# cosmir17/Scala-akka-tensorflow-sharetrade-helper

Measured on AMD Instinct MI355X. Metric: env steps/sec (whole node) + episode return, 2x128 MLP Q-net at 1/2/4/8 MI355X, higher is better.
Workload: dtype bf16; 1 GPU; model=2x128 MLP Q-net (203->128->128->3), online DQN, Adam, global_batch=1835008, seq_len=201, parallelism=dp1, dp_gradient_sync=none, envs_per_gpu=1835008, hip_graph=True, graph_steps=16, kernel_chunk=64, step_kernel=ws, chunk_schedule=static

## Files before the change

csrc/qtarget.hip:

```cpp
#include "qstep.h"

namespace st {
namespace qtgt {

constexpr int INP = 224, HP = 128, KX = 208, HWIN = 201;

constexpr int KS = 208;
constexpr int oW0 = 0;
constexpr int oW1 = oW0 + HP * KS * 2;
constexpr int oW2 = oW1 + HP * HP * 2;
constexpr int oB1 = oW2 + 4 * HP * 2;
constexpr int LDS_BYTES = oB1 + HP * 4;

ST_DEV int w1_off(int r, int c) { return r * HP + ((((c >> 3) ^ (r & 15))) << 3) + (c & 7); }
ST_DEV f4v mfma32z(s4v a, s4v b, f4v c) {
  const s4v z = {0, 0, 0, 0};
  return mfma32(cat8(a, z), cat8(b, z), c);
}
struct QTargetParams {
  const float* prices4;
  const int* env;
  const float* wt;
  float* qt;
  int T, E, T4;
  int off_w0, off_w1, off_b1, off_w2, off_b2;
  float b0, inv_b0;
  int s0, compat_env, output_relu, feat_mode;
  const unsigned char* wimg;
  const unsigned short* ticks;
  const float* tscale;
  int T16;
};

template <int FEAT, int TPW, int NWV, bool U16 = false>
__global__ void __launch_bounds__(64 * NWV, 1) qtarget_kernel(QTargetParams p) {
  static_assert(!U16 || FEAT, "the tick bank serves the relative features only");
  constexpr int NW = NWV, NT = 64 * NWV;
  extern __shared__ __attribute__((aligned(16))) char smem[];
  bf16_t* W0 = reinterpret_cast<bf16_t*>(smem + oW0);
  bf16_t* W1 = reinterpret_cast<bf16_t*>(smem + oW1);
  bf16_t* W2 = reinterpret_cast<bf16_t*>(smem + oW2);
  float* B1 = reinterpret_cast<float*>(smem + oB1);
  const int tid = threadIdx.x, lane = tid & 63, l16 = lane & 15, g4 = lane >> 4;
  const int w = tid >> 6;
  if (p.wimg != nullptr) {
    constexpr int NCH = LDS_BYTES / 16;
    const int lane_ = tid & 63;
    for (int j = tid >> 6; j * 64 < NCH; j += NW) {
      const int c = j * 64 + lane_;
      if (c < NCH)
        __builtin_amdgcn_global_load_lds((const __attribute__((address_space(1))) void*)(p.wimg + 16 * c),
                                         (__attribute__((address_space(3))) void*)(smem + 1024 * j), 16, 0, 0);
    }
    __builtin_amdgcn_s_waitcnt(0xF70);
  } else {
  for (int i = tid; i < HP * KX; i += NT) {
    const int r = i / KX, s = i % KX;
    W0[r * KS + s] = f2bf(p.wt[p.off_w0 + r * INP + slot_col(s)]);
  }
  for (int i = tid; i < HP * HP; i += NT) {
    const int r = i / HP, s = i % HP;
    W1[w1_off(r, s)] = f2bf(p.wt[p.off_w1 + r * HP + pi_unit(s)]);
  }
  for (int i = tid; i < 4 * HP; i += NT) {
    const int a = i / HP, s = i % HP;
    W2[i] = a < 3 ? f2bf(p.wt[p.off_w2 + a * HP + pi_unit(s)]) : (bf16_t)0;
  }
  for (int i = tid; i < HP; i += NT) B1[i] = p.wt[p.off_b1 + i];
  }
  __syncthreads();
  const float b2v[3] = {p.wt[p.off_b2], p.wt[p.off_b2 + 1], p.wt[p.off_b2 + 2]};
  const size_t E = (size_t)p.E;
  const int ntiles = p.E / 16;
  s4v w0t[8];
#pragma unroll
  for (int i = 0; i < 8; ++i) w0t[i] = lds_ld4(W0 + (16 * i + l16) * KS + 192 + 4 * g4);
  for (int t0 = (blockIdx.x * NW + w) * TPW; t0 < ntiles; t0 += gridDim.x * NW * TPW) {
    int zo = 0;
    asm volatile("" : "+s"(zo));
    const bf16_t* W0i = W0 + zo;
    float vnew[TPW], invn[TPW], vnw[TPW];
    Holding hd[TPW];
    s8v X[TPW][6];
    s4v Xw[TPW];
#pragma unroll
    for (int q = 0; q < TPW; ++q) {
      const int e = 16 * (t0 + q) + l16;
      const int pos = p.env[ER_POS * E + e];
      const float bud = __int_as_float(p.env[ER_BUDGET * E + e]);
      const int sh = p.env[ER_SHARES * E + e];
      const int pc = min(max(pos, 0), p.T - HWIN - 1);
      if (U16) {
        const unsigned* b = reinterpret_cast<const unsigned*>(p.ticks + (size_t)e * p.T16) + ((pc + 1) >> 1);
        const unsigned shb = (unsigned)((pc + 1) & 1) * 2u;
        const unsigned tv = __builtin_amdgcn_alignbyte(0u, b[100], shb);
        const float vw = (float)(tv & 0xFFFFu);
        vnew[q] = __fmul_rn(vw, p.tscale[e]);
        invn[q] = __fdiv_rn(1.0f, vw);
        vnw[q] = vw;
        const float iv = invn[q];
        auto fxn = [&](float v) { return __fmaf_rn(v, iv, -1.0f); };
        auto lo16f = [](unsigned v) { return (float)(v & 0xFFFFu); };
        auto hi16f = [](unsigned v) { return (float)(v >> 16); };
#pragma unroll
        for (int ks = 0; ks < 6; ++ks) {
          uint4 u;
          __builtin_memcpy(&u, b + 16 * ks + 4 * g4, sizeof(u));
          const unsigned t4 = b[16 * ks + 4 * g4 + 4];
          const unsigned w0 = __builtin_amdgcn_alignbyte(u.y, u.x, shb), w1 = __builtin_amdgcn_alignbyte(u.z, u.y, shb),
                         w2 = __builtin_amdgcn_alignbyte(u.w, u.z, shb), w3 = __builtin_amdgcn_alignbyte(t4, u.w, shb);
          X[q][ks] = cat8(pk4(fxn(lo16f(w0)), fxn(hi16f(w0)), fxn(lo16f(w1)), fxn(hi16f(w1))),
                          pk4(fxn(lo16f(w2)), fxn(hi16f(w2)), fxn(lo16f(w3)), fxn(hi16f(w3))));
        }
        Xw[q] = s4v{0, 0, 0, 0};
        if (g4 == 1 || g4 == 2) {
          uint2 u;
          __builtin_memcpy(&u, b + 96 + 2 * (g4 - 1), sizeof(u));
          const unsigned t2 = b[98 + 2 * (g4 - 1)];
          const unsigned w0 = __builtin_amdgcn_alignbyte(u.y, u.x, shb), w1 = __builtin_amdgcn_alignbyte(t2, u.y, shb);
          Xw[q] = pk4(fxn(lo16f(w0)), fxn(hi16f(w0)), fxn(lo16f(w1)), fxn(hi16f(w1)));
        }
      } else {
      const float* b = p.prices4 + (size_t)e * p.T4 + (size_t)pc;
      vnew[q] = b[201];
      vnw[q] = vnew[q];
      invn[q] = FEAT ? __fdiv_rn(1.0f, vnew[q]) : 0.f;
      const float iv = invn[q];
      auto fxn = [&](float v) { return FEAT ? __fmaf_rn(v, iv, -1.0f) : v; };
#pragma unroll
      for (int ks = 0; ks < 6; ++ks) {
        const float4 u = ldu4(b + 1 + 32 * ks + 8 * g4), v = ldu4(b + 5 + 32 * ks + 8 * g4);
        X[q][ks] = cat8(pk4(fxn(u.x), fxn(u.y), fxn(u.z), fxn(u.w)), pk4(fxn(v.x), fxn(v.y), fxn(v.z), fxn(v.w)));
      }
      Xw[q] = s4v{0, 0, 0, 0};
      if (g4 == 1 || g4 == 2) {
        const float4 u = ldu4(b + 193 + 4 * (g4 - 1));
        Xw[q] = pk4(fxn(u.x), fxn(u.y), fxn(u.z), fxn(u.w));
      }
      }
      hd[q] = trade_base(bud, sh, p.compat_env, p.b0, p.s0);
    }
    f4v a1[TPW][8];
#pragma unroll
    for (int i = 0; i < 8; ++i) {
#pragma unroll
      for (int q = 0; q < TPW; ++q) a1[q][i] = f4v{0.f, 0.f, 0.f, 0.f};
      const bf16_t* wr = W0i + (16 * i + l16) * KS + 8 * g4;
#pragma unroll
      for (int ks = 0; ks < 6; ++ks) {
        const s8v A = lds_ld8(wr + 32 * ks);
#pragma unroll
        for (int q = 0; q < TPW; ++q) a1[q][i] = mfma32(A, X[q][ks], a1[q][i]);
      }
#pragma unroll
      for (int q = 0; q < TPW; ++q) a1[q][i] = mfma32z(w0t[i], Xw[q], a1[q][i]);
    }
#pragma unroll 1
    for (int a = 0; a < 3; ++a) {
      int za = 0;
      asm volatile("" : "+s"(za));
      const bf16_t* W1a = W1 + za;
      const bf16_t* W2a = W2 + za;
      s8v H1[TPW][4];
#pragma unroll
      for (int q = 0; q < TPW; ++q) {
        const Holding h2 = trade(a, hd[q], vnew[q]);
        const float fvn = FEAT ? __fmaf_rn(vnw[q], invn[q], -1.0f) : vnew[q];
        const s4v tl = g4 == 0 ? pk4(feat_budget(h2.budget, p.inv_b0, FEAT),
                                     feat_shares(h2.shares, vnew[q], p.inv_b0, FEAT), 1.0f, fvn)
                               : s4v{0, 0, 0, 0};
#pragma unroll
        for (int ks = 0; ks < 4; ++ks) {
          const f4v z0 = mfma32z(w0t[2 * ks], tl, a1[q][2 * ks]);
          const f4v z1 = mfma32z(w0t[2 * ks + 1], tl, a1[q][2 * ks + 1]);
          H1[q][ks] = cat8(relu_bf(z0), relu_bf(z1));
        }
      }
      f4v qo[TPW];
#pragma unroll
      for (int q = 0; q < TPW; ++q) qo[q] = f4v{0.f, 0.f, 0.f, 0.f};
      const bf16_t* w2r = W2a + min(l16, 3) * HP + 8 * g4;
#pragma unroll
      for (int ks2 = 0; ks2 < 4; ++ks2) {
        f4v z[TPW][2];
#pragma unroll
        for (int h = 0; h < 2; ++h) {
          const int i = 2 * ks2 + h;
          const f4v bias = *reinterpret_cast<const f4v*>(B1 + 16 * i + 4 * g4);
#pragma unroll
          for (int q = 0; q < TPW; ++q) z[q][h] = bias;
#pragma unroll
          for (int ks = 0; ks < 4; ++ks) {
            const s8v A = lds_ld8(W1a + w1_off(16 * i + l16, 32 * ks + 8 * g4));
#pragma unroll
            for (int q = 0; q < TPW; ++q) z[q][h] = mfma32(A, H1[q][ks], z[q][h]);
          }
        }
        const s8v A2 = lds_ld8(w2r + 32 * ks2);
#pragma unroll
        for (int q = 0; q < TPW; ++q) qo[q] = mfma32(A2, cat8(relu_bf(z[q][0]), relu_bf(z[q][1])), qo[q]);
      }
      if (g4 == 0) {
#pragma unroll
        for (int q = 0; q < TPW; ++q) {
          float o[3];
#pragma unroll
          for (int j = 0; j < 3; ++j) {
            o[j] = qo[q][j] + b2v[j];
            if (p.output_relu) o[j] = fmaxf(o[j], 0.f);
          }
          const int e = 16 * (t0 + q) + l16;
          *reinterpret_cast<float4*>(p.qt + ((size_t)e * 3 + a) * 4) = make_float4(o[0], o[1], o[2], 0.f);
        }
      }
    }
  }
}

__global__ void __launch_bounds__(256) qt_img_map_kernel(int* map, int off_w0, int off_w1, int off_w2, int off_b1) {
  const int i = blockIdx.x * blockDim.x + threadIdx.x;
  if (i < HP * KX) map[off_w0 + (i / KX) * INP + slot_col(i % KX)] = oW0 / 2 + (i / KX) * KS + i % KX;
  if (i < HP * HP) map[off_w1 + (i / HP) * HP + pi_unit(i % HP)] = oW1 / 2 + w1_off(i / HP, i % HP);
  if (i < 3 * HP) map[off_w2 + (i / HP) * HP + pi_unit(i % HP)] = oW2 / 2 + i;
  if (i < HP) map[off_b1 + i] = -(oB1 / 4 + i) - 2;
}

}
}

extern "C" int st_qtarget_img_bytes() { return st::qtgt::LDS_BYTES; }

extern "C" hipError_t st_qtarget_img_map(int* map, int off_w0, int off_w1, int off_w2, int off_b1, hipStream_t stream) {
  using namespace st::qtgt;
  static_assert(LDS_BYTES % 16 == 0 && oW0 == 0, "image run");
  hipLaunchKernelGGL(qt_img_map_kernel, dim3((HP * KX + 255) / 256), dim3(256), 0, stream, map, off_w0, off_w1, off_w2,
                     off_b1);
  return hipGetLastError();
}


namespace {
template <int TPW, int NWV>
hipError_t launch_qt(const st::qtgt::QTargetParams* p, int grid, hipStream_t stream) {
  using namespace st::qtgt;
  if (p->E % (16 * TPW) != 0) return hipErrorInvalidValue;
  static bool attr[3] = {false, false, false};
  const bool u16 = p->ticks != nullptr;
  if (u16 && (!p->feat_mode || p->tscale == nullptr || p->T16 < p->T + 8 || p->T16 % 8)) return hipErrorInvalidValue;
  const int f = u16 ? 2 : (p->feat_mode ? 1 : 0);
  const void* fn = f == 2 ? (const void*)qtarget_kernel<1, TPW, NWV, true>
                          : (f ? (const void*)qtarget_kernel<1, TPW, NWV> : (const void*)qtarget_kernel<0, TPW, NWV>);
  if (!attr[f]) {
    hipError_t e = hipFuncSetAttribute(fn, hipFuncAttributeMaxDynamicSharedMemorySize, LDS_BYTES);
    if (e != hipSuccess) return e;
    attr[f] = true;
  }
  if (f == 2)
    hipLaunchKernelGGL((qtarget_kernel<1, TPW, NWV, true>), dim3(grid), dim3(64 * NWV), LDS_BYTES, stream, *p);
  else if (f)
    hipLaunchKernelGGL((qtarget_kernel<1, TPW, NWV>), dim3(grid), dim3(64 * NWV), LDS_BYTES, stream, *p);
  else
    hipLaunchKernelGGL((qtarget_kernel<0, TPW, NWV>), dim3(grid), dim3(64 * NWV), LDS_BYTES, stream, *p);
  return hipGetLastError();
}
}

extern "C" hipError_t st_qtarget_launch_v(const st::qtgt::QTargetParams* p, int grid, int variant, hipStream_t stream) {
  using namespace st::qtgt;
  if (grid < 1 || p->T < HWIN + 2 || p->T4 < p->T + 4) return hipErrorInvalidValue;
  switch (variant) {
    case 0: return launch_qt<4, 4>(p, grid, stream);
    case 1: return launch_qt<2, 8>(p, grid, stream);
    case 2: return launch_qt<1, 8>(p, grid, stream);
    case 3: return launch_qt<1, 16>(p, grid, stream);
    default: return hipErrorInvalidValue;
  }
}
extern "C" hipError_t st_qtarget_launch(const st::qtgt::QTargetParams* p, int grid, hipStream_t stream) {
  return st_qtarget_launch_v(p, grid, 1, stream);
}

extern "C" int st_abi_qtarget(int* out, int n) {
  const int sz[] = {(int)sizeof(st::QStepParams), (int)sizeof(st::qtgt::QTargetParams)};
  const int m = (int)(sizeof(sz) / sizeof(sz[0]));
  for (int i = 0; i < n && i < m; ++i) out[i] = sz[i];
  return m;
}
```

sharetrade/ops/native.py:

```python
from __future__ import annotations

import ctypes as C
import os
from typing import Optional

import torch

_HERE = os.path.dirname(os.path.abspath(__file__))
LIB_DIR = os.path.join(os.path.dirname(_HERE), "_native")
HIP_LIB_PATH = os.path.join(LIB_DIR, "libsharetrade_hip.so")

_lib: Optional[C.CDLL] = None


class NativeUnavailable(RuntimeError):
    pass


class QStepParams(C.Structure):
    _fields_ = [
        ("prices", C.c_void_p), ("prices4", C.c_void_p), ("env", C.c_void_p),
        ("wq", C.c_void_p), ("wf", C.c_void_p), ("slab", C.c_void_p), ("stats", C.c_void_p), ("ctrl", C.c_void_p),
        ("T", C.c_int), ("E", C.c_int), ("H", C.c_int), ("P", C.c_int), ("T4", C.c_int),
        ("off_w0", C.c_int), ("off_w1", C.c_int), ("off_b1", C.c_int), ("off_w2", C.c_int), ("off_b2", C.c_int),
        ("eps", C.c_float), ("inv_ramp", C.c_float), ("gamma", C.c_float), ("loss_coef", C.c_float),
        ("b0", C.c_float), ("inv_b0", C.c_float),
        ("s0", C.c_int), ("compat_env", C.c_int), ("target_compat", C.c_int), ("output_relu", C.c_int),
        ("feat_mode", C.c_int),
        ("key0", C.c_uint32), ("key1", C.c_uint32),
        ("env_offset", C.c_int),
        ("stamps", C.c_void_p),
        ("slab_bf16", C.c_int), ("slab_rows", C.c_int),
        ("chunk_heads", C.c_void_p),
        ("reward_mode", C.c_int), ("td_clip", C.c_float),
        ("err", C.c_void_p),
        ("reward_scale", C.c_float), ("ramp_global", C.c_int), ("qt", C.c_void_p), ("double_dqn", C.c_int),
        ("wimg", C.c_void_p),
        ("ticks", C.c_void_p), ("tscale", C.c_void_p), ("T16", C.c_int),
    ]


QTARGET_VARIANTS = {0: (4, 4), 1: (2, 8), 2: (1, 8), 3: (1, 16)}


class QTargetParams(C.Structure):
    _fields_ = [
        ("prices4", C.c_void_p), ("env", C.c_void_p), ("wt", C.c_void_p), ("qt", C.c_void_p),
        ("T", C.c_int), ("E", C.c_int), ("T4", C.c_int),
        ("off_w0", C.c_int), ("off_w1", C.c_int), ("off_b1", C.c_int), ("off_w2", C.c_int), ("off_b2", C.c_int),
        ("b0", C.c_float), ("inv_b0", C.c_float),
        ("s0", C.c_int), ("compat_env", C.c_int), ("output_relu", C.c_int), ("feat_mode", C.c_int),
        ("wimg", C.c_void_p),
        ("ticks", C.c_void_p), ("tscale", C.c_void_p), ("T16", C.c_int),
    ]


class OptimParams(C.Structure):
    _fields_ = [
        ("params", C.c_void_p), ("params_bf", C.c_void_p), ("mask", C.c_void_p), ("s1", C.c_void_p),
        ("s2", C.c_void_p), ("slab", C.c_void_p), ("grad", C.c_void_p), ("ctrl", C.c_void_p),
        ("stats", C.c_void_p), ("stat_acc", C.c_void_p),
        ("G", C.c_int), ("P", C.c_int), ("kind", C.c_int), ("mode", C.c_int), ("nstat", C.c_int),
        ("lr", C.c_float), ("beta1", C.c_float), ("beta2", C.c_float), ("eps", C.c_float), ("scale", C.c_float),
        ("tdelay", C.c_int), ("slab_bf16", C.c_int),
        ("chunk_heads", C.c_void_p),
        ("ema", C.c_void_p), ("ema_decay", C.c_float),
        ("img_map", C.c_void_p), ("img", C.c_void_p),
    ]


REWARD_MODES = {"absolute": 0, "relative": 1, "growth": 2}

ENV_ROWS = ("pos", "budget", "shares", "value", "ret_sum", "episodes", "last_final", "actions_out", "rewards_out")


AB_LIB_PATH = os.path.join(LIB_DIR, "libsharetrade_ab.so")
WRONG_RESULT_VARIANTS = frozenset({"gskip", "gskipst", "l1x2", "l2x2", "nopf", "nowb", "nophil"})
_ab_lib: Optional[C.CDLL] = None


def ab_builds_enabled() -> bool:
    return os.environ.get("SHARETRADE_AB_BUILDS", "") not in ("", "0")


def ab_lib() -> C.CDLL:
    global _ab_lib
    if not ab_builds_enabled():
        raise RuntimeError("timing / debug kernel builds are opt-in: set SHARETRADE_AB_BUILDS=1 and run "
                           "`python build.py --ab` (csrc/ab/*.hip -> libsharetrade_ab.so)")
    if _ab_lib is None:
        if not os.path.exists(AB_LIB_PATH):
            raise NativeUnavailable(f"{AB_LIB_PATH} not built: run `SHARETRADE_AB_BUILDS=1 python build.py`")
        lib()
        _ab_lib = C.CDLL(AB_LIB_PATH)
    return _ab_lib


def variant_launch(suffix: str, prefix: str = "st_qstep_ws_launch_"):
    if not ab_builds_enabled():
        bad = " (computes WRONG results by design)" if suffix in WRONG_RESULT_VARIANTS else ""
        raise RuntimeError(f"engine.step_variant={suffix!r}{bad} needs SHARETRADE_AB_BUILDS=1")
    fn = getattr(ab_lib(), prefix + suffix)
    fn.argtypes = [C.POINTER(QStepParams), C.c_int, C.c_int, C.c_int, C.c_int, C.c_void_p]
    fn.restype = C.c_int
    return fn


def available() -> bool:
    return os.path.exists(HIP_LIB_PATH)


def lib() -> C.CDLL:
    global _lib
    if _lib is not None:
        return _lib
    if not os.path.exists(HIP_LIB_PATH):
        raise NativeUnavailable(
            f"{HIP_LIB_PATH} not built: run `python build.py` (hipcc --offload-arch=gfx950)")
    L = C.CDLL(HIP_LIB_PATH)
    L.st_qstep_launch.argtypes = [C.POINTER(QStepParams), C.c_int, C.c_int, C.c_int, C.c_int, C.c_void_p]
    L.st_qstep_launch.restype = C.c_int
    L.st_qstep_lds_bytes.argtypes = [C.c_int, C.c_int, C.c_int]
    L.st_qstep_lds_bytes.restype = C.c_int
    L.st_qstep_wide_launch.argtypes = [C.POINTER(QStepParams), C.c_int, C.c_int, C.c_int, C.c_int, C.c_void_p]
    L.st_qstep_wide_launch.restype = C.c_int
    L.st_qstep_wide_lds_bytes.argtypes = [C.c_int, C.c_int, C.c_int]
    L.st_qstep_wide_lds_bytes.restype = C.c_int
    L.st_qstep_wide_launch_w8.argtypes = [C.POINTER(QStepParams), C.c_int, C.c_int, C.c_int, C.c_int, C.c_void_p]
    L.st_qstep_wide_launch_w8.restype = C.c_int
    L.st_qstep_ws_launch.argtypes = [C.POINTER(QStepParams), C.c_int, C.c_int, C.c_int, C.c_int, C.c_void_p]
    L.st_qstep_ws_launch.restype = C.c_int
    L.st_qstep_ws_lds_bytes.argtypes = [C.c_int, C.c_int, C.c_int]
    L.st_qstep_ws_lds_bytes.restype = C.c_int
    L.st_qtarget_launch.argtypes = [C.POINTER(QTargetParams), C.c_int, C.c_void_p]
    L.st_qtarget_launch.restype = C.c_int
    L.st_qtarget_launch_v.argtypes = [C.POINTER(QTargetParams), C.c_int, C.c_int, C.c_void_p]
    L.st_qtarget_launch_v.restype = C.c_int
    L.st_qtarget_img_bytes.argtypes = []
    L.st_qtarget_img_bytes.restype = C.c_int
    L.st_qtarget_img_map.argtypes = [C.c_void_p] + [C.c_int] * 4 + [C.c_void_p]
    L.st_qtarget_img_map.restype = C.c_int
    L.st_f32b_target_sync.argtypes = [C.c_void_p, C.c_void_p, C.c_longlong, C.c_void_p, C.c_longlong, C.c_void_p]
    L.st_f32b_target_sync.restype = C.c_int
    L.st_reduce_optim.argtypes = [C.POINTER(OptimParams), C.c_void_p]
    L.st_reduce_optim.restype = C.c_int
    L.st_advance.argtypes = [C.c_void_p, C.c_void_p]
    L.st_advance.restype = C.c_int
    L.st_commit_step.argtypes = [C.c_void_p, C.c_void_p]
    L.st_commit_step.restype = C.c_int
    L.st_to_bf16.argtypes = [C.c_void_p, C.c_void_p, C.c_int, C.c_void_p]
    L.st_to_bf16.restype = C.c_int
    L.st_img_pack.argtypes = [C.c_void_p, C.c_void_p, C.c_void_p, C.c_int, C.c_void_p]
    L.st_img_pack.restype = C.c_int
    L.st_qstep_ws_img_bytes.argtypes = []
    L.st_qstep_ws_img_bytes.restype = C.c_int
    L.st_qstep_ws_img_map.argtypes = [C.c_void_p] + [C.c_int] * 5 + [C.c_void_p]
    L.st_qstep_ws_img_map.restype = C.c_int
    L.st_random_walk.argtypes = [C.c_void_p, C.c_int, C.c_int, C.c_float, C.c_float, C.c_float, C.c_uint32,
                                 C.c_uint32, C.c_void_p]
    L.st_random_walk.restype = C.c_int
    L.st_replicate4.argtypes = [C.c_void_p, C.c_void_p, C.c_int, C.c_int, C.c_int, C.c_int, C.c_void_p]
    L.st_replicate4.restype = C.c_int
    L.st_tick16.argtypes = [C.c_void_p, C.c_int, C.c_int, C.c_void_p, C.c_int, C.c_void_p, C.c_int, C.c_void_p,
                            C.c_void_p]
    L.st_tick16.restype = C.c_int
    L.st_init_normal.argtypes = [C.c_void_p, C.c_int, C.c_int, C.c_int, C.c_float, C.c_uint32, C.c_uint32,
                                 C.c_uint32, C.c_void_p]
    L.st_init_normal.restype = C.c_int
    _bind_optional(L)
    _lib = L
    return L


def _bind_optional(L: C.CDLL) -> None:
    if hasattr(L, "st_occupy"):
        L.st_occupy.argtypes = [C.c_int, C.c_int, C.c_void_p, C.c_void_p]
        L.st_occupy.restype = C.c_int
    if hasattr(L, "st_tick_rcp_table"):
        L.st_tick_rcp_table.argtypes = [C.c_void_p, C.c_void_p, C.c_void_p]
        L.st_tick_rcp_table.restype = C.c_int
    if hasattr(L, "st_mlp_fwd_f32"):
        L.st_mlp_fwd_f32.restype = C.c_int
        L.st_td_update_f32.restype = C.c_int


def clear_last_error() -> int:
    return int(C.CDLL("libamdhip64.so").hipGetLastError())


def check(err: int, what: str) -> None:
    if err != 0:
        raise RuntimeError(f"HIP error {err} in {what}")


def ptr(t: Optional[torch.Tensor]) -> Optional[int]:
    if t is None:
        return None
    return t.data_ptr()


def stream_handle() -> int:
    return torch.cuda.current_stream().cuda_stream


def qstep_supported(inp: int, h1p: int, h2p: int) -> bool:
    if not available():
        return False
    return lib().st_qstep_lds_bytes(inp, h1p, h2p) > 0


def qstep_wide_supported(inp: int, h1p: int, h2p: int) -> bool:
    if not available():
        return False
    return lib().st_qstep_wide_lds_bytes(inp, h1p, h2p) > 0


def qstep_ws_supported(inp: int, h1p: int, h2p: int) -> bool:
    if not available():
        return False
    return lib().st_qstep_ws_lds_bytes(inp, h1p, h2p) > 0


def qstep_pipe_supported(inp: int, h1p: int, h2p: int) -> bool:
    if not available():
        return False
    fn = ab_lib().st_qstep_pipe_lds_bytes
    fn.argtypes = [C.c_int, C.c_int, C.c_int]
    fn.restype = C.c_int
    return fn(inp, h1p, h2p) > 0


def random_walk(out: torch.Tensor, start_price: float, vol: float, drift: float, key0: int, key1: int) -> None:
    E, T = out.shape
    check(lib().st_random_walk(ptr(out), E, T, start_price, vol, drift, key0 & 0xFFFFFFFF, key1 & 0xFFFFFFFF,
                               stream_handle()), "st_random_walk")


def replica_stride(T: int) -> int:
    return (T + 64 + 3) // 4 * 4


def replicate4(src: torch.Tensor, reps: int = 4) -> torch.Tensor:
    E, T = src.shape
    T4 = replica_stride(T)
    flat = torch.zeros(reps * E * T4 + 64, dtype=torch.float32, device=src.device)
    out = flat[: reps * E * T4].view(reps, E, T4)
    check(lib().st_replicate4(ptr(src), ptr(out), E, T, T4, int(reps), stream_handle()), "st_replicate4")
    return out


def tick16_stride(T: int) -> int:
    return (T + 8 + 7) // 8 * 8


def tick16(bank: torch.Tensor, quantize: bool):
    E, T = bank.shape
    if not bank.is_contiguous():
        raise ValueError("tick16: contiguous [E, T] bank expected")
    T16 = tick16_stride(T)
    flat = torch.zeros(E * T16 + 64, dtype=torch.int16, device=bank.device)
    ticks = flat[: E * T16].view(E, T16)
    scale = torch.empty(E, dtype=torch.float32, device=bank.device)
    bad = torch.zeros(1, dtype=torch.int32, device=bank.device)
    check(lib().st_tick16(ptr(bank), E, T, ptr(ticks), T16, ptr(scale), 0 if quantize else 1, ptr(bad),
                          stream_handle()), "st_tick16")
    if not quantize and int(bad.item()) != 0:
        return None
    return ticks, scale


def tick_rcp_table(device) -> tuple:
    div = torch.zeros(65535, dtype=torch.int32, device=device)
    rcp = torch.ones(65535, dtype=torch.int32, device=device)
    check(lib().st_tick_rcp_table(ptr(div), ptr(rcp), stream_handle()), "st_tick_rcp_table")
    return div, rcp


def tick16_quantize_(bank: torch.Tensor) -> torch.Tensor:
    E, T = bank.shape
    if not bank.is_contiguous():
        raise ValueError("tick16: contiguous [E, T] bank expected")
    check(lib().st_tick16(ptr(bank), E, T, None, 0, None, 0, None, stream_handle()), "st_tick16")
    return bank


def init_normal(block: torch.Tensor, rows: int, cols: int, std: float, key0: int, key1: int, stream: int) -> None:
    if not block.is_cuda or block.dtype != torch.float32 or block.dim() != 2 or block.stride(1) != 1:
        raise ValueError("init_normal: a 2-D row-major fp32 CUDA view is required")
    if rows > block.shape[0] or cols > block.shape[1]:
        raise ValueError("init_normal: block too small")
# ... 31 lines not shown
```

sharetrade/trainer/engine.py:

```python
from __future__ import annotations

import contextlib

import math
import os
import time
from typing import Dict, Optional

import numpy as np
import torch

from ..config import Config
from ..env import trading as tr
from ..models import qnet as qn
from ..ops import native
from ..utils import rng
from .graphs import CAPTURE_MODE

NSTAT = 8
STAT_NAMES = ("reward_sum", "loss_sum", "explore", "episodes_done", "final_sum", "final_sq", "qslot_sum", "_")
OPT_KIND = {"sgd": 0, "adagrad": 1, "adam": 2}


def resolve_device(spec: str) -> torch.device:
# ... 195 lines not shown
        self.opt = qn.OptimState(a.optimizer, L.numel, a.adagrad_init_acc, device=self.device)
        self.state = tr.EnvState.create(self.E, cfg.env.budget, cfg.env.shares, device=self.device)
        self.env_offset = rank * self.E
        self.step_count = 0
        self.key0, self.key1 = rng.key_for(a.seed, 0)
        total = self.E * world_size
        self.loss_coef = 2.0 / total if a.loss_reduction == "mean" else 2.0
        self.stats = torch.zeros(NSTAT, dtype=torch.float64)
        self._sync = None
        if world_size > 1:
            from ..parallel.dist import DistContext, GradSync

            ctx = DistContext(rank, world_size, 0, "dist", self.device, group)
            self._sync = GradSync(ctx, L.numel, bucket_mb=cfg.engine.bucket_mb,
                                  compress=cfg.engine.grad_compress or None)
        self._graph = None
        self._last_actions: Optional[torch.Tensor] = None
        if be == "native":
            self._init_native()

    def ws_ok(self, cfg: Config, L) -> bool:
        return (self.E % 64 == 0 and self.H == 201 and tuple(L.pdims[:3]) == (224, 128, 128)
                and native.qstep_ws_supported(L.pdims[0], L.pdims[1], L.pdims[2]))

    def _init_native(self):
        dev = self.device
        L = self.layout
        self.ctrl = torch.zeros(2, dtype=torch.int64, device=dev)
        self.env_soa = torch.zeros(len(native.ENV_ROWS), self.E, dtype=torch.int32, device=dev)
        rows = {}
        for i, k in enumerate(native.ENV_ROWS):
            src = getattr(self.state, k, None)
            dt = torch.float32 if k in ("budget", "value", "ret_sum", "last_final", "rewards_out") else torch.int32
            rows[k] = self.env_soa[i].view(dt)
            if src is not None:
                rows[k].copy_(src)
        for k in self.state.as_dict():
            setattr(self.state, k, rows[k])
        self.actions_out, self.rewards_out = rows["actions_out"], rows["rewards_out"]
        self.grad = torch.zeros(L.numel, dtype=torch.float32, device=dev)
        self.stat_acc = torch.zeros(NSTAT, dtype=torch.float64, device=dev)
        if self.kernel == "fp32_rows":
            from ..ops.mlp_f32 import F32BatchedStep, F32EngineStep

            fb = self.cfg.engine.f32_batched
            if fb not in ("auto", "on", "off"):
                raise ValueError(f"engine.f32_batched: {fb!r}")
            self.f32_path = "batched" if (fb == "on" or (fb == "auto" and self.E >= 1024)) else "rows"
            if self._learn_knobs and self.f32_path != "batched":
                raise NotImplementedError("the learning-experiment knobs need the batched fp32 step "
                                          "(engine.f32_batched='on', or 'auto' with >= 1,024 envs)")
            self._f32 = F32BatchedStep(self) if self.f32_path == "batched" else F32EngineStep(self)
            return
        self.params_bf = torch.empty(L.numel, dtype=torch.bfloat16, device=dev)
        self.ticks = self.tscale = None
        b16 = self.cfg.engine.bank16
        if b16 not in ("auto", "off"):
            raise ValueError(f"engine.bank16: {b16!r}")
        if (b16 == "auto" and self.step_kernel == "ws" and self.cfg.env.features == "relative"
                and self.prices.is_contiguous()):
            t16 = native.tick16(self.prices, quantize=False)
            if t16 is not None:
                self.ticks, self.tscale = t16
        self.prices4 = (None if self.ticks is not None else
                        native.replicate4(self.prices, 1 if self.step_kernel in ("ws", "pipe") else 4))
        self._wimg = self._wimg_map = None
        if self.step_kernel == "ws" and os.environ.get("SHARETRADE_WS_WIMG", "1") != "0":
            self._wimg, self._wimg_map = native.ws_weight_image(self.params, self.layout.segments)
        self._bf16_refresh()
        props = torch.cuda.get_device_properties(dev)
        self.grid = max(1, min(self.cfg.engine.grid or props.multi_processor_count, self.E // self.chunk))
        self.slab_bf16 = (self.chunk == 64 and self.cfg.engine.slab_dtype == "bf16" and L.numel % 32 == 0
                          and all(seg.offset % 32 == 0 for seg in L.segments.values()))
        self.slab = (torch.zeros((L.numel + 127) // 128 * 128 * self.grid, dtype=torch.bfloat16, device=dev)
                     if self.slab_bf16 else torch.zeros(self.grid, L.numel, dtype=torch.float32, device=dev))
        self.stat_slab = torch.zeros(self.grid, NSTAT, dtype=torch.float32, device=dev)
        sched = self.cfg.engine.chunk_schedule
        if sched == "auto":
            sched = ("dynamic" if (self.world_size > 1 and self.cfg.engine.dp_overlap and self.step_kernel != "ws")
                     else "static")
        if sched not in ("static", "dynamic"):
            raise ValueError(f"engine.chunk_schedule: {sched!r}")
        if sched == "dynamic" and self.step_kernel == "ws" and self._learn_knobs:
            raise ValueError("engine.chunk_schedule='dynamic' is not available with the learning knobs "
                             "(agent.target_every / double_dqn / reward_scale / ramp_mode) on the ws kernel; "
                             "use 'static' or 'auto'")
        dyn_ok = ((self.step_kernel == "wide" and self.grid % 8 == 0 and (self.E // 64) % 8 == 0)
                  or (self.step_kernel == "ws" and self.grid % 8 == 0))
        self.chunk_schedule = "dynamic" if (sched == "dynamic" and dyn_ok) else "static"
        self.chunk_heads = (torch.zeros(8 * 32, dtype=torch.int32, device=dev)
                            if self.chunk_schedule == "dynamic" else None)
        self.qt_buf = None
        if self.cfg.agent.target_every:
            self.params_target = self.params.detach().clone()
            self.qt_buf = torch.zeros(self.E * 12, dtype=torch.float32, device=dev)
        self._build_structs()

    def _build_structs(self):
        cfg, L, st = self.cfg, self.layout, self.state
        seg = L.segments
        q = native.QStepParams()
        if self.prices4 is not None:
            q.prices4, q.T4 = native.ptr(self.prices4), int(self.prices4.shape[2])
        else:
            q.prices4, q.T4 = None, native.replica_stride(self.T)
        if self.ticks is not None:
            q.ticks, q.tscale, q.T16 = native.ptr(self.ticks), native.ptr(self.tscale), int(self.ticks.shape[1])
        q.prices, q.env = native.ptr(self.prices), native.ptr(self.env_soa)
        q.wq, q.wf = native.ptr(self.params_bf), native.ptr(self.params)
        q.wimg = native.ptr(self._wimg) if self._wimg is not None else None
        q.slab, q.stats = native.ptr(self.slab), native.ptr(self.stat_slab)
        q.slab_bf16, q.slab_rows = int(self.slab_bf16), self.grid
        q.ctrl = native.ptr(self.ctrl)
        q.T, q.E, q.H, q.P = self.T, self.E, self.H, L.numel
        q.off_w0, q.off_w1, q.off_b1 = seg["W0"].offset, seg["W1"].offset, seg["b1"].offset
        q.off_w2, q.off_b2 = seg["W2"].offset, seg["b2"].offset
        q.eps = cfg.agent.epsilon
        q.inv_ramp = float(np.float32(1.0 / cfg.agent.ramp))
        q.gamma = cfg.agent.gamma
        q.loss_coef = self.loss_coef
        q.b0 = cfg.env.budget
        q.inv_b0 = float(np.float32(1.0 / cfg.env.budget))
        q.s0 = cfg.env.shares
        q.compat_env = int(cfg.env.compat_decisions)
        q.target_compat = int(cfg.agent.target_slot == "compat")
        q.output_relu = int(cfg.model.output_relu)
        q.feat_mode = tr.FEATURES[cfg.env.features]
        q.key0, q.key1 = int(self.key0), int(self.key1)
        q.env_offset = self.env_offset
        q.chunk_heads = native.ptr(self.chunk_heads) if self.chunk_heads is not None else None
        q.reward_mode = native.REWARD_MODES[cfg.agent.reward_mode]
        q.td_clip = float(cfg.agent.td_clip)
        self.kernel_err = torch.zeros(4, dtype=torch.int32, device=self.device)
        q.err = native.ptr(self.kernel_err)
        a = cfg.agent
        q.reward_scale = float(a.reward_scale)
        q.ramp_global = int(a.ramp_mode == "global")
        q.double_dqn = int(a.double_dqn)
        q.qt = native.ptr(self.qt_buf) if self.qt_buf is not None else None
        self._qp = q
        self._qtp = None
        if self.qt_buf is not None:
            t = native.QTargetParams()
            t.prices4, t.env, t.wt, t.qt = q.prices4, q.env, native.ptr(self.params_target), q.qt
            t.T, t.E, t.T4 = q.T, q.E, q.T4
            t.ticks, t.tscale, t.T16 = q.ticks, q.tscale, q.T16
            t.off_w0, t.off_w1, t.off_b1, t.off_w2, t.off_b2 = q.off_w0, q.off_w1, q.off_b1, q.off_w2, q.off_b2
            t.b0, t.inv_b0, t.s0 = q.b0, q.inv_b0, q.s0
            t.compat_env, t.output_relu, t.feat_mode = q.compat_env, q.output_relu, q.feat_mode
            if os.environ.get("SHARETRADE_WS_WIMG", "1") != "0":
                self._qt_img, self._qt_map = native.qtarget_weight_image(self.params_target, seg)
                t.wimg = native.ptr(self._qt_img)
            self._qtp = t
            self._qt_variant = int(os.environ.get("SHARETRADE_QT_VARIANT", "3"))
            tpw, nw = native.QTARGET_VARIANTS[self._qt_variant]
            if self.E % (16 * tpw):
                raise NotImplementedError(f"target pass: E % {16 * tpw} != 0")
            self._qt_grid = max(1, min(torch.cuda.get_device_properties(self.device).multi_processor_count,
                                       self.E // (16 * tpw * nw)))
        a = cfg.agent
        o = native.OptimParams()
        o.params, o.params_bf, o.mask = native.ptr(self.params), native.ptr(self.params_bf), native.ptr(self.mask)
        if self._wimg is not None:
            o.img, o.img_map = native.ptr(self._wimg), native.ptr(self._wimg_map)
        o.s1 = native.ptr(self.opt.s1) if self.opt.s1.numel() else None
        o.s2 = native.ptr(self.opt.s2) if self.opt.s2.numel() else None
        o.slab, o.grad, o.ctrl = native.ptr(self.slab), native.ptr(self.grad), native.ptr(self.ctrl)
        o.slab_bf16 = int(self.slab_bf16)
        o.G, o.P, o.kind = self.grid, L.numel, OPT_KIND[a.optimizer]
        o.stats, o.stat_acc, o.nstat = native.ptr(self.stat_slab), native.ptr(self.stat_acc), NSTAT
        o.lr, o.beta1, o.beta2, o.eps, o.scale = a.lr, a.adam_betas[0], a.adam_betas[1], a.adam_eps, 1.0
        o.chunk_heads = q.chunk_heads
        if self.params_ema is not None:
            o.ema, o.ema_decay = native.ptr(self.params_ema), self.ema_decay
        self._op = o

    def _native_step(self):
        if self.kernel == "fp32_rows":
            ar = None
            if self.world_size > 1:
                ar = self._sync.all_reduce
            self._f32.step(self.grad, ar)
            self._f32_stats()
            self._ema_update()
            return
        L = native.lib()
        sh = native.stream_handle()
        if self.world_size > 1 and self.cfg.engine.dp_overlap:
            self._launch_qstep(L, sh)
            self._overlap_step(L, sh)
            self._target_sync(L, sh)
        elif self.world_size > 1:
            self._dp_pre()
            self._sync.all_reduce(self.grad)
            self._dp_post()
        else:
            self._launch_qstep(L, sh)
            self._op.mode = 0
            native.check(L.st_reduce_optim(self._op, sh), "reduce_optim")
            self._target_sync(L, sh)

    def _dp_pre(self) -> None:
        L, sh = native.lib(), native.stream_handle()
        self._launch_qstep(L, sh)
        self._op.mode = 1
        native.check(L.st_reduce_optim(self._op, sh), "reduce")

    def _dp_post(self) -> None:
        L, sh = native.lib(), native.stream_handle()
        self._op.mode = 2
        native.check(L.st_reduce_optim(self._op, sh), "update")
        self._target_sync(L, sh)

    def _target_sync(self, L, sh) -> None:
        if self._qtp is not None:
            native.check(L.st_f32b_target_sync(native.ptr(self.params), native.ptr(self.params_target),
                                               self.params.numel(), native.ptr(self.ctrl),
                                               int(self.cfg.agent.target_every), sh), "target_sync")

    def _target_img_refresh(self) -> None:
        if getattr(self, "_qt_img", None) is not None:
            native.img_pack(self.params_target, self._qt_map, self._qt_img)

    def _launch_qstep(self, L, sh) -> None:
        if self._qtp is not None:
            self._target_img_refresh()
            native.check(L.st_qtarget_launch_v(self._qtp, self._qt_grid, self._qt_variant, sh), "qtarget")
        if self.step_kernel == "pipe":
            fn = native.variant_launch(self.cfg.engine.step_variant, "st_qstep_pipe_launch_") \
                if self.cfg.engine.step_variant else native.variant_launch("", "st_qstep_pipe_launch")
        elif self.step_kernel == "ws":
            fn = L.st_qstep_ws_launch
            if self._qp.stamps:
                fn = native.variant_launch(self.cfg.engine.step_variant or "stamps")
            elif self.cfg.engine.step_variant:
                fn = native.variant_launch(self.cfg.engine.step_variant)
        elif self.chunk == 64:
            fn = L.st_qstep_wide_launch_w8 if self.cfg.engine.step_waves == 8 else L.st_qstep_wide_launch
        else:
            fn = L.st_qstep_launch
        d = self.layout.pdims
        native.check(fn(self._qp, d[0], d[1], d[2], self.grid, sh), f"qstep(chunk={self.chunk})")

    def _overlap_step(self, L, sh) -> None:
        if not hasattr(self, "_ov"):
            import ctypes as C

            bufs = [self.grad, torch.zeros_like(self.grad)]
            ops = []
            for b in bufs:
                o = native.OptimParams()
                C.pointer(o)[0] = self._op
                o.grad = native.ptr(b)
                o.tdelay = 1
                ops.append(o)
            self._ov = {"bufs": bufs, "ops": ops, "parity": 0, "pending": None}
        ov = self._ov
        i = ov["parity"]
        op = ov["ops"][i]
        op.mode = 1
        native.check(L.st_reduce_optim(op, sh), "reduce")
        wait_new = self._sync.start(ov["bufs"][i])
        if ov["pending"] is not None:
            wait_prev, j = ov["pending"]
            wait_prev()
            upd = ov["ops"][j]
            upd.mode = 2
            native.check(L.st_reduce_optim(upd, sh), "update")
        else:
            native.check(L.st_commit_step(native.ptr(self.ctrl), sh), "commit")
        ov["pending"] = (wait_new, i)
        ov["parity"] = i ^ 1

    def flush_pending(self) -> None:
        ov = getattr(self, "_ov", None)
        if ov is None or ov["pending"] is None:
            return
        wait_prev, j = ov["pending"]
        wait_prev()
        upd = ov["ops"][j]
        upd.mode, upd.tdelay = 2, 0
        L, sh = native.lib(), native.stream_handle()
        native.check(L.st_reduce_optim(upd, sh), "update")
        upd.tdelay = 1
        ov["pending"] = None
        self._target_sync(L, sh)

    def _f32_stats(self) -> None:
        if getattr(self._f32, "stats_in_kernel", False):
            return
        r = self.rewards_out.double()
        self.stat_acc[0] += r.sum()
        self.stat_acc[1] += self._f32.s.loss.double().sum()

    def native_grad(self) -> torch.Tensor:
        if self.kernel == "fp32_rows":
            self._f32.grad(self.grad)
            self._f32_stats()
            self.step_count += 1
            return self.grad
        L = native.lib()
        sh = native.stream_handle()
        self._launch_qstep(L, sh)
        self._op.mode = 1
        native.check(L.st_reduce_optim(self._op, sh), "reduce")
        self.step_count += 1
        return self.grad

# ... 290 lines not shown
```

Baseline: 3.091 billion env_steps/s.

## Add joint-action target-Q kernel variant and make it the default

Adds a JOINT template path in the target-Q kernel that evaluates all three actions together. Each W1 and W2 fragment is loaded from LDS once and reused across the three actions, instead of being reloaded in a per-action loop. For 16-wave blocks the layer-0 tail weights (w0t) are reloaded from LDS inside the tile loop rather than held in registers across it, to ease register pressure. The default variant changes to the joint 1x16 configuration. In exchange, the joint path holds H1, z and qo for three actions at once, which raises register use and risks spills.

```diff
diff --git a/csrc/qtarget.hip b/csrc/qtarget.hip
--- a/csrc/qtarget.hip
+++ b/csrc/qtarget.hip
@@ -32,7 +32,7 @@
   int T16;
 };
 
-template <int FEAT, int TPW, int NWV, bool U16 = false>
+template <int FEAT, int TPW, int NWV, bool U16 = false, bool JOINT = false>
 __global__ void __launch_bounds__(64 * NWV, 1) qtarget_kernel(QTargetParams p) {
   static_assert(!U16 || FEAT, "the tick bank serves the relative features only");
   constexpr int NW = NWV, NT = 64 * NWV;
@@ -72,9 +72,12 @@
   const float b2v[3] = {p.wt[p.off_b2], p.wt[p.off_b2 + 1], p.wt[p.off_b2 + 2]};
   const size_t E = (size_t)p.E;
   const int ntiles = p.E / 16;
+  constexpr bool PT = JOINT && NWV >= 16;
   s4v w0t[8];
+  if constexpr (!PT) {
 #pragma unroll
   for (int i = 0; i < 8; ++i) w0t[i] = lds_ld4(W0 + (16 * i + l16) * KS + 192 + 4 * g4);
+  }
   for (int t0 = (blockIdx.x * NW + w) * TPW; t0 < ntiles; t0 += gridDim.x * NW * TPW) {
     int zo = 0;
     asm volatile("" : "+s"(zo));
@@ -140,6 +143,10 @@
       }
       hd[q] = trade_base(bud, sh, p.compat_env, p.b0, p.s0);
     }
+    if constexpr (PT) {
+#pragma unroll
+      for (int i = 0; i < 8; ++i) w0t[i] = lds_ld4(W0i + (16 * i + l16) * KS + 192 + 4 * g4);
+    }
     f4v a1[TPW][8];
 #pragma unroll
     for (int i = 0; i < 8; ++i) {
@@ -155,6 +162,7 @@
 #pragma unroll
       for (int q = 0; q < TPW; ++q) a1[q][i] = mfma32z(w0t[i], Xw[q], a1[q][i]);
     }
+    if constexpr (!JOINT) {
 #pragma unroll 1
     for (int a = 0; a < 3; ++a) {
       int za = 0;
@@ -214,6 +222,98 @@
         }
       }
     }
+    } else {
+      int za = 0;
+      asm volatile("" : "+s"(za));
+      const bf16_t* W1a = W1 + za;
+      const bf16_t* W2a = W2 + za;
+      s4v tl[3][TPW];
+#pragma unroll
+      for (int a = 0; a < 3; ++a) {
+#pragma unroll
+        for (int q = 0; q < TPW; ++q) {
+          const Holding h2 = trade(a, hd[q], vnew[q]);
+          const float fvn = FEAT ? __fmaf_rn(vnw[q], invn[q], -1.0f) : vnew[q];
+          tl[a][q] = g4 == 0 ? pk4(feat_budget(h2.budget, p.inv_b0, FEAT),
+                                   feat_shares(h2.shares, vnew[q], p.inv_b0, FEAT), 1.0f, fvn)
+                             : s4v{0, 0, 0, 0};
+        }
+      }
+      s8v H1[3][TPW][4];
+#pragma unroll
+      for (int ks = 0; ks < 4; ++ks) {
+#pragma unroll
+        for (int a = 0; a < 3; ++a) {
+#pragma unroll
+          for (int q = 0; q < TPW; ++q) {
+            const f4v z0 = mfma32z(w0t[2 * ks], tl[a][q], a1[q][2 * ks]);
+            const f4v z1 = mfma32z(w0t[2 * ks + 1], tl[a][q], a1[q][2 * ks + 1]);
+            H1[a][q][ks] = cat8(relu_bf(z0), relu_bf(z1));
+          }
+        }
+      }
+      f4v qo[3][TPW];
+#pragma unroll
+      for (int a = 0; a < 3; ++a) {
+#pragma unroll
+        for (int q = 0; q < TPW; ++q) qo[a][q] = f4v{0.f, 0.f, 0.f, 0.f};
+      }
+      const bf16_t* w2r = W2a + min(l16, 3) * HP + 8 * g4;
+#pragma unroll
+      for (int ks2 = 0; ks2 < 4; ++ks2) {
+        s4v zp[3][TPW];
+#pragma unroll
+        for (int h = 0; h < 2; ++h) {
+          const int i = 2 * ks2 + h;
+          const f4v bias = *reinterpret_cast<const f4v*>(B1 + 16 * i + 4 * g4);
+          f4v z[3][TPW];
+#pragma unroll
+          for (int a = 0; a < 3; ++a) {
+#pragma unroll
+            for (int q = 0; q < TPW; ++q) z[a][q] = bias;
+          }
+#pragma unroll
+          for (int ks = 0; ks < 4; ++ks) {
+            const s8v A = lds_ld8(W1a + w1_off(16 * i + l16, 32 * ks + 8 * g4));
+#pragma unroll
+            for (int a = 0; a < 3; ++a) {
+#pragma unroll
+              for (int q = 0; q < TPW; ++q) z[a][q] = mfma32(A, H1[a][q][ks], z[a][q]);
+            }
+          }
+          if (h == 0) {
+#pragma unroll
+            for (int a = 0; a < 3; ++a) {
+#pragma unroll
+              for (int q = 0; q < TPW; ++q) zp[a][q] = relu_bf(z[a][q]);
+            }
+          } else {
+            const s8v A2 = lds_ld8(w2r + 32 * ks2);
+#pragma unroll
+            for (int a = 0; a < 3; ++a) {
+#pragma unroll
+              for (int q = 0; q < TPW; ++q) qo[a][q] = mfma32(A2, cat8(zp[a][q], relu_bf(z[a][q])), qo[a][q]);
+            }
+          }
+        }
+      }
+      if (g4 == 0) {
+#pragma unroll
+        for (int a = 0; a < 3; ++a) {
+#pragma unroll
+          for (int q = 0; q < TPW; ++q) {
+            float o[3];
+#pragma unroll
+            for (int j = 0; j < 3; ++j) {
+              o[j] = qo[a][q][j] + b2v[j];
+              if (p.output_relu) o[j] = fmaxf(o[j], 0.f);
+            }
+            const int e = 16 * (t0 + q) + l16;
+            *reinterpret_cast<float4*>(p.qt + ((size_t)e * 3 + a) * 4) = make_float4(o[0], o[1], o[2], 0.f);
+          }
+        }
+      }
+    }
   }
 }
 
@@ -240,7 +340,7 @@
 
 
 namespace {
-template <int TPW, int NWV>
+template <int TPW, int NWV, bool JOINT = false>
 hipError_t launch_qt(const st::qtgt::QTargetParams* p, int grid, hipStream_t stream) {
   using namespace st::qtgt;
   if (p->E % (16 * TPW) != 0) return hipErrorInvalidValue;
@@ -248,33 +348,50 @@
   const bool u16 = p->ticks != nullptr;
   if (u16 && (!p->feat_mode || p->tscale == nullptr || p->T16 < p->T + 8 || p->T16 % 8)) return hipErrorInvalidValue;
   const int f = u16 ? 2 : (p->feat_mode ? 1 : 0);
-  const void* fn = f == 2 ? (const void*)qtarget_kernel<1, TPW, NWV, true>
-                          : (f ? (const void*)qtarget_kernel<1, TPW, NWV> : (const void*)qtarget_kernel<0, TPW, NWV>);
+  const void* fn = f == 2 ? (const void*)qtarget_kernel<1, TPW, NWV, true, JOINT>
+                          : (f ? (const void*)qtarget_kernel<1, TPW, NWV, false, JOINT> : (const void*)qtarget_kernel<0, TPW, NWV, false, JOINT>);
   if (!attr[f]) {
     hipError_t e = hipFuncSetAttribute(fn, hipFuncAttributeMaxDynamicSharedMemorySize, LDS_BYTES);
     if (e != hipSuccess) return e;
     attr[f] = true;
   }
   if (f == 2)
-    hipLaunchKernelGGL((qtarget_kernel<1, TPW, NWV, true>), dim3(grid), dim3(64 * NWV), LDS_BYTES, stream, *p);
+    hipLaunchKernelGGL((qtarget_kernel<1, TPW, NWV, true, JOINT>), dim3(grid), dim3(64 * NWV), LDS_BYTES, stream, *p);
   else if (f)
-    hipLaunchKernelGGL((qtarget_kernel<1, TPW, NWV>), dim3(grid), dim3(64 * NWV), LDS_BYTES, stream, *p);
+    hipLaunchKernelGGL((qtarget_kernel<1, TPW, NWV, false, JOINT>), dim3(grid), dim3(64 * NWV), LDS_BYTES, stream, *p);
   else
-    hipLaunchKernelGGL((qtarget_kernel<0, TPW, NWV>), dim3(grid), dim3(64 * NWV), LDS_BYTES, stream, *p);
+    hipLaunchKernelGGL((qtarget_kernel<0, TPW, NWV, false, JOINT>), dim3(grid), dim3(64 * NWV), LDS_BYTES, stream, *p);
   return hipGetLastError();
 }
 }
 
+namespace {
+constexpr int QT_VARIANTS[][3] = {{4, 4, 0}, {2, 8, 0}, {1, 8, 0}, {1, 16, 0}, {1, 8, 1}, {1, 12, 1}, {1, 16, 1}};
+constexpr int N_QT_VARIANTS = (int)(sizeof(QT_VARIANTS) / sizeof(QT_VARIANTS[0]));
+template <int V>
+hipError_t launch_variant(const st::qtgt::QTargetParams* p, int grid, hipStream_t stream) {
+  return launch_qt<QT_VARIANTS[V][0], QT_VARIANTS[V][1], QT_VARIANTS[V][2] != 0>(p, grid, stream);
+}
+}
 extern "C" hipError_t st_qtarget_launch_v(const st::qtgt::QTargetParams* p, int grid, int variant, hipStream_t stream) {
   using namespace st::qtgt;
   if (grid < 1 || p->T < HWIN + 2 || p->T4 < p->T + 4) return hipErrorInvalidValue;
+  static_assert(N_QT_VARIANTS == 7, "one case per table row");
   switch (variant) {
-    case 0: return launch_qt<4, 4>(p, grid, stream);
-    case 1: return launch_qt<2, 8>(p, grid, stream);
-    case 2: return launch_qt<1, 8>(p, grid, stream);
-    case 3: return launch_qt<1, 16>(p, grid, stream);
+    case 0: return launch_variant<0>(p, grid, stream);
+    case 1: return launch_variant<1>(p, grid, stream);
+    case 2: return launch_variant<2>(p, grid, stream);
+    case 3: return launch_variant<3>(p, grid, stream);
+    case 4: return launch_variant<4>(p, grid, stream);
+    case 5: return launch_variant<5>(p, grid, stream);
+    case 6: return launch_variant<6>(p, grid, stream);
     default: return hipErrorInvalidValue;
   }
+}
+extern "C" int st_qtarget_variants(int* out, int n) {
+  for (int v = 0; v < N_QT_VARIANTS && v < n; ++v)
+    for (int j = 0; j < 3; ++j) out[3 * v + j] = QT_VARIANTS[v][j];
+  return N_QT_VARIANTS;
 }
 extern "C" hipError_t st_qtarget_launch(const st::qtgt::QTargetParams* p, int grid, hipStream_t stream) {
   return st_qtarget_launch_v(p, grid, 1, stream);
diff --git a/sharetrade/ops/native.py b/sharetrade/ops/native.py
--- a/sharetrade/ops/native.py
+++ b/sharetrade/ops/native.py
@@ -40,7 +40,9 @@
     ]
 
 
-QTARGET_VARIANTS = {0: (4, 4), 1: (2, 8), 2: (1, 8), 3: (1, 16)}
+QTARGET_VARIANTS = {0: (4, 4, False), 1: (2, 8, False), 2: (1, 8, False), 3: (1, 16, False),
+                    4: (1, 8, True), 5: (1, 12, True), 6: (1, 16, True)}
+QTARGET_DEFAULT = 6
 
 
 class QTargetParams(C.Structure):
@@ -136,6 +138,8 @@
     L.st_qtarget_launch.restype = C.c_int
     L.st_qtarget_launch_v.argtypes = [C.POINTER(QTargetParams), C.c_int, C.c_int, C.c_void_p]
     L.st_qtarget_launch_v.restype = C.c_int
+    L.st_qtarget_variants.argtypes = [C.POINTER(C.c_int), C.c_int]
+    L.st_qtarget_variants.restype = C.c_int
     L.st_qtarget_img_bytes.argtypes = []
     L.st_qtarget_img_bytes.restype = C.c_int
     L.st_qtarget_img_map.argtypes = [C.c_void_p] + [C.c_int] * 4 + [C.c_void_p]
diff --git a/sharetrade/trainer/engine.py b/sharetrade/trainer/engine.py
--- a/sharetrade/trainer/engine.py
+++ b/sharetrade/trainer/engine.py
@@ -371,8 +371,8 @@
                 self._qt_img, self._qt_map = native.qtarget_weight_image(self.params_target, seg)
                 t.wimg = native.ptr(self._qt_img)
             self._qtp = t
-            self._qt_variant = int(os.environ.get("SHARETRADE_QT_VARIANT", "3"))
-            tpw, nw = native.QTARGET_VARIANTS[self._qt_variant]
+            self._qt_variant = int(os.environ.get("SHARETRADE_QT_VARIANT", native.QTARGET_DEFAULT))
+            tpw, nw, _ = native.QTARGET_VARIANTS[self._qt_variant]
             if self.E % (16 * tpw):
                 raise NotImplementedError(f"target pass: E % {16 * tpw} != 0")
             self._qt_grid = max(1, min(torch.cuda.get_device_properties(self.device).multi_processor_count,
```

Measured after the change: 3.091 billion env_steps/s. No clear change (-0.0%).
